# aikiriao/AAD

Hardware: AMD Instinct MI355X
Metric: Msamples/s encode+decode, 48 kHz stereo 4-bit (higher is better)
Workload: dtype int32

## Files before the change

### aad_amd/capi.py

```python
import ctypes as C
import os

import numpy as np


class AADApiResult:
    OK = 0
    INVALID_ARGUMENT = 1
    INVALID_FORMAT = 2
    INSUFFICIENT_BUFFER = 3
    INSUFFICIENT_DATA = 4
    PARAMETER_NOT_SET = 5
    NG = 6
    _names = {0: "OK", 1: "INVALID_ARGUMENT", 2: "INVALID_FORMAT", 3: "INSUFFICIENT_BUFFER",
              4: "INSUFFICIENT_DATA", 5: "PARAMETER_NOT_SET", 6: "NG"}

    @classmethod
    def name(cls, v):
        return cls._names.get(int(v), str(v))


class AADHeaderInfo(C.Structure):
    _fields_ = [("format_version", C.c_uint32), ("codec_version", C.c_uint32),
                ("num_channels", C.c_uint16), ("num_samples", C.c_uint32),
# ... 11 lines not shown
class AADHipStreamDesc(C.Structure):
    _fields_ = [("pcm_offset", C.c_uint64), ("data_offset", C.c_uint64),
                ("data_size", C.c_uint64), ("num_samples", C.c_uint32), ("reserved", C.c_uint32)]


class AADHipSegmentation(C.Structure):
    _fields_ = [("segment_blocks", C.c_uint32), ("warmup_blocks", C.c_uint32)]


class AADHipPlanarLayout(C.Structure):
    _fields_ = [("sample_type", C.c_int32), ("reserved", C.c_uint32), ("channel_stride", C.c_uint64)]


class AADHipPlanarOutput(C.Structure):
    _fields_ = [("sample_type", C.c_int32), ("reserved", C.c_uint32), ("stream_stride", C.c_uint64), ("channel_stride", C.c_uint64)]


class AADHipRowStats(C.Structure):
    _fields_ = [("sum_sq", C.c_uint64), ("sum_abs", C.c_uint64), ("max_abs", C.c_uint64), ("count", C.c_uint64)]


class AADHipLaneState(C.Structure):
    _fields_ = [("weight", C.c_int32 * 4), ("history", C.c_int32 * 4),
                ("stepsize_index", C.c_int32), ("quantize_error", C.c_int32)]


STREAM_DESC_DTYPE = np.dtype([("pcm_offset", "<u8"), ("data_offset", "<u8"), ("data_size", "<u8"),
                              ("num_samples", "<u4"), ("reserved", "<u4")])
ERROR_STATS_DTYPE = np.dtype([("rms_error", "<f8"), ("mean_abs_error", "<f8"), ("max_abs_error", "<f8")])
WINDOW_DTYPE = np.dtype([("stream", "<i8"), ("first_frame", "<i8")])
SAMPLE_INT16, SAMPLE_FLOAT32 = 0, 1
RECONSTRUCT_DECODED, RECONSTRUCT_RESIDUAL = 0, 1
OPTION_LANE_MAPPING, OPTION_TRIAL_LANES, OPTION_STAGING_THREADS, OPTION_TILE_KBYTES, OPTION_COMPARE_ORDER = 0, 1, 2, 3, 4
LANE_MAPPINGS = {"auto": 0, "dense": 1, "quad": 2, "quad-fused": 3, "dense-tiled": 4}
TRIAL_LANES = {"dual": 0, "single": 1}
LANE_STATE_DTYPE = np.dtype([("weight", "<i4", (4,)), ("history", "<i4", (4,)),
                             ("stepsize_index", "<i4"), ("quantize_error", "<i4")])

_PKG_DIR = os.path.dirname(os.path.abspath(__file__))
LIBRARY_PATH = os.environ.get("AAD_HIP_LIBRARY", os.path.join(_PKG_DIR, "libaad_hip.so"))

LEGACY_SYMBOLS = [
    "AADEncoder_CalculateBlockSize", "AADEncoder_EncodeHeader", "AADEncoder_CalculateWorkSize",
    "AADEncoder_Create", "AADEncoder_Destroy", "AADEncoder_SetEncodeParameter", "AADEncoder_EncodeWhole",
    "AADDecoder_DecodeHeader", "AADDecoder_CalculateWorkSize", "AADDecoder_Create", "AADDecoder_Destroy",
    "AADDecoder_SetHeader", "AADDecoder_DecodeBlock", "AADDecoder_DecodeWhole",
]
HIP_SYMBOLS = [
    "AADHip_GetDeviceCount", "AADHip_ContextCreate", "AADHip_ContextDestroy", "AADHip_ContextSynchronize",
    "AADHip_ContextLastError", "AADHip_ContextSignalNextRun", "AADHip_SignalNextRunSupported", "AADHip_ContextSetOption", "AADHip_CalculateEncodedSize", "AADHip_EncodePlanCreate",
    "AADHip_EncodePlanDestroy", "AADHip_EncodePlanRun", "AADHip_DecodePlanCreate", "AADHip_DecodePlanDestroy",
    "AADHip_DecodePlanRun", "AADHip_EncodeBatch", "AADHip_DecodeBatch",
    "AADHip_ReconstructPlanCreate", "AADHip_ReconstructPlanDestroy", "AADHip_ReconstructPlanRun",
    "AADHip_ReconstructBatch", "AADHip_SegmentedEncodePlanCreate", "AADHip_SegmentedEncodeBatch",
    "AADHip_SegmentedReconstructPlanCreate", "AADHip_SegmentedReconstructBatch",
    "AADHip_WindowDecodePlanCreate", "AADHip_WindowDecodePlanDestroy", "AADHip_WindowDecodePlanRun",
    "AADHip_PlanarEncodePlanCreate", "AADHip_PlanarEncodePlanRun",
    "AADHip_PlanarReconstructPlanCreate", "AADHip_PlanarReconstructPlanRun", "AADHip_PlanarReconstructPlanRunStats",
]
WAV_SYMBOLS = ["AADWav_ParseHeader", "AADWav_WriteHeader", "AADWav_ConvertToPcm16"]
SYNTH_SYMBOLS = ["AADSynth_Generate"]


class AADWavInfo(C.Structure):
    _fields_ = [("format_tag", C.c_uint16), ("num_channels", C.c_uint16), ("sampling_rate", C.c_uint32),
                ("bits_per_sample", C.c_uint16), ("num_samples", C.c_uint32), ("data_offset", C.c_uint64),
                ("data_size", C.c_uint64)]


def _declare_legacy(lib):
    u8p, i32pp = C.POINTER(C.c_uint8), C.POINTER(C.POINTER(C.c_int32))
    lib.AADEncoder_CalculateBlockSize.argtypes = [C.c_uint16, C.c_uint16, C.c_uint32,
                                                  C.POINTER(C.c_uint16), C.POINTER(C.c_uint32)]
    lib.AADEncoder_CalculateBlockSize.restype = C.c_int
    lib.AADEncoder_EncodeHeader.argtypes = [C.POINTER(AADHeaderInfo), u8p, C.c_uint32]
    lib.AADEncoder_EncodeHeader.restype = C.c_int
    lib.AADEncoder_CalculateWorkSize.argtypes = [C.c_uint16]
    lib.AADEncoder_CalculateWorkSize.restype = C.c_int32
    lib.AADEncoder_Create.argtypes = [C.c_uint16, C.c_void_p, C.c_int32]
    lib.AADEncoder_Create.restype = C.c_void_p
    lib.AADEncoder_Destroy.argtypes = [C.c_void_p]
    lib.AADEncoder_Destroy.restype = None
    lib.AADEncoder_SetEncodeParameter.argtypes = [C.c_void_p, C.POINTER(AADEncodeParameter)]
    lib.AADEncoder_SetEncodeParameter.restype = C.c_int
    lib.AADEncoder_EncodeWhole.argtypes = [C.c_void_p, i32pp, C.c_uint32, u8p, C.c_uint32, C.POINTER(C.c_uint32)]
    lib.AADEncoder_EncodeWhole.restype = C.c_int
    lib.AADDecoder_DecodeHeader.argtypes = [u8p, C.c_uint32, C.POINTER(AADHeaderInfo)]
    lib.AADDecoder_DecodeHeader.restype = C.c_int
    lib.AADDecoder_CalculateWorkSize.argtypes = []
    lib.AADDecoder_CalculateWorkSize.restype = C.c_int32
    lib.AADDecoder_Create.argtypes = [C.c_void_p, C.c_int32]
# ... 54 lines not shown
    lib.AADHip_DecodePlanCreate.argtypes = [vp, C.POINTER(AADHeaderInfo), C.c_int32, C.c_uint32, vp, C.POINTER(vp)]
    lib.AADHip_DecodePlanCreate.restype = C.c_int
    lib.AADHip_DecodePlanDestroy.argtypes = [vp]
    lib.AADHip_DecodePlanDestroy.restype = None
    lib.AADHip_DecodePlanRun.argtypes = [vp, vp, vp]
    lib.AADHip_DecodePlanRun.restype = C.c_int
    lib.AADHip_WindowDecodePlanCreate.argtypes = [vp, C.POINTER(AADHeaderInfo), C.c_int32, C.c_uint32, vp, C.POINTER(vp)]
    lib.AADHip_WindowDecodePlanCreate.restype = C.c_int
    lib.AADHip_WindowDecodePlanDestroy.argtypes = [vp]
    lib.AADHip_WindowDecodePlanDestroy.restype = None
    lib.AADHip_WindowDecodePlanRun.argtypes = [vp, vp, C.c_uint64, vp, C.c_uint32, C.c_int32, vp]
    lib.AADHip_WindowDecodePlanRun.restype = C.c_int
    lib.AADHip_EncodeBatch.argtypes = [vp, C.POINTER(AADEncodeParameter), C.c_uint32, vp, vp, vp, vp, vp, vp]
    lib.AADHip_EncodeBatch.restype = C.c_int
    lib.AADHip_DecodeBatch.argtypes = [vp, C.c_uint32, vp, vp, vp, vp, vp]
    lib.AADHip_DecodeBatch.restype = C.c_int
    lib.AADHip_ReconstructPlanCreate.argtypes = [vp, C.POINTER(AADEncodeParameter), C.c_uint32, vp, C.POINTER(vp)]
    lib.AADHip_ReconstructPlanCreate.restype = C.c_int
    lib.AADHip_ReconstructPlanDestroy.argtypes = [vp]
    lib.AADHip_ReconstructPlanDestroy.restype = None
    lib.AADHip_ReconstructPlanRun.argtypes = [vp, vp, vp, vp, C.c_int32, vp]
    lib.AADHip_ReconstructPlanRun.restype = C.c_int
    lib.AADHip_ReconstructBatch.argtypes = [vp, C.POINTER(AADEncodeParameter), C.c_uint32, vp, vp, C.c_int32, vp, vp]
    lib.AADHip_ReconstructBatch.restype = C.c_int
    lib.AADHip_SegmentedEncodeBatch.argtypes = [vp, C.POINTER(AADEncodeParameter), C.POINTER(AADHipSegmentation), C.c_uint32, vp, vp,
                                                vp, vp, vp]
    lib.AADHip_SegmentedEncodeBatch.restype = C.c_int
    lib.AADHip_SegmentedReconstructPlanCreate.argtypes = [vp, C.POINTER(AADEncodeParameter), C.POINTER(AADHipSegmentation), C.c_uint32,
                                                          vp, C.POINTER(vp)]
    lib.AADHip_SegmentedReconstructPlanCreate.restype = C.c_int
    lib.AADHip_SegmentedReconstructBatch.argtypes = [vp, C.POINTER(AADEncodeParameter), C.POINTER(AADHipSegmentation), C.c_uint32, vp,
                                                     vp, C.c_int32, vp, vp]
    lib.AADHip_SegmentedReconstructBatch.restype = C.c_int
    lib.AADWav_ParseHeader.argtypes = [vp, C.c_uint64, C.POINTER(AADWavInfo)]
    lib.AADWav_ParseHeader.restype = C.c_int
    lib.AADWav_WriteHeader.argtypes = [vp, C.c_uint32, C.c_uint16, C.c_uint32, C.c_uint32]
    lib.AADWav_WriteHeader.restype = C.c_int
    lib.AADWav_ConvertToPcm16.argtypes = [vp, C.c_uint16, C.c_uint64, vp]
    lib.AADWav_ConvertToPcm16.restype = C.c_int


def load_library(path=None, hip=True):
    path = path or LIBRARY_PATH
    if not os.path.exists(path):
        raise FileNotFoundError(
            "%s is missing - the HIP extension has not been built (run __graft_entry__.build())" % path)
    if hip:
        try:
            import torch
        except ImportError:
            pass
    lib = C.CDLL(path)
    _declare_legacy(lib)
    if hip:
        _declare_hip(lib)
    return lib


def make_parameter(channels, bits, max_block_size=1024, rate=48000, ms=False, trials=0):
    return AADEncodeParameter(num_channels=channels, sampling_rate=rate, bits_per_sample=bits,
                              max_block_size=max_block_size, ch_process_method=1 if ms else 0,
                              num_encode_trials=trials)


def _planar_pointers(planar):
    rows = (C.POINTER(C.c_int32) * planar.shape[0])()
# ... 88 lines not shown
```

### aad_amd/csrc/aad_hip_engine.hip

```cpp
#include <hip/hip_runtime.h>

#include <cstdio>
#include <cstdlib>
#include <cstring>
#include <algorithm>
#include <condition_variable>
#include <functional>
#include <mutex>
#include <new>
#include <thread>
#include <vector>

#include "../../include/aad_hip.h"
#include "aad_compare.hip.h"
#include "aad_launch.h"
#include "aad_decode.hip.h"
#include "aad_decode_window.hip.h"
#include "aad_encode.hip.h"
#include "aad_encode_launch.hip.h"
#include "aad_format.h"
#include "aad_hip_internal.h"
#include "aad_tiles.h"

namespace aad {
// ... 12 lines not shown
struct StagingPool {
  std::vector<std::thread> threads;
  std::mutex lock;
  std::condition_variable work, done;
  std::function<void(unsigned)> job;
  unsigned generation = 0, pending = 0;
  bool stop = false;
};

struct AADHipContext {
  int device;
  hipStream_t stream;
  bool owns_stream;
  char last_error[256];
  Staging in[2], out[2];
  hipEvent_t chunk_done[2];
  hipEvent_t piece_done[3];
  hipStream_t up_stream, down_stream;
  hipEvent_t uploaded[2], computed[2];
  bool have_events, have_pipeline;
  void *d_rc_in, *d_rc_out;
  size_t rc_in_capacity, rc_out_capacity;
  void *d_scratch;
  size_t scratch_capacity;
  int32_t *d_residual;
  uint64_t residual_capacity;
  uint8_t *d_trial;
  uint64_t trial_capacity;
  aad::LaunchSignal signal_next;
  bool signal_refused;
  aad::Device device_info;
  aad::Knobs knobs;
  int32_t compare_sequential;
  int64_t tile_bytes;
  void *d_state;
  size_t state_capacity;
  int32_t staging_threads;
  StagingPool *pool;
};

enum class EncodePlanKind {
  Frames,
  Rows,
  Reconstruct
};

struct AADHipEncodePlan {
  AADHipContext *ctx;
  EncodePlanKind kind;
  aad::EncodeRun run;
  void *d_table;
  uint64_t *d_out_base;
  uint32_t *d_stats_stream;
  uint64_t stats_records;
};

struct AADHipDecodePlan {
  AADHipContext *ctx;
  aad::DecodeArgs args;
  aad::StreamDesc *d_streams;
  uint64_t *d_prefix;
};

struct AADHipWindowDecodePlan {
  AADHipContext *ctx;
  aad::DecodeArgs args;
// ... 563 lines not shown
      if (ctx->d_trial) (void)hipFree(ctx->d_trial);
      if (ctx->d_state) (void)hipFree(ctx->d_state);
      if (ctx->owns_stream) (void)hipStreamDestroy(ctx->stream);
    }
  }
  delete ctx;
}

AADApiResult AADHip_ContextSynchronize(struct AADHipContext *ctx)
{
  if (ctx == nullptr) return AAD_APIRESULT_INVALID_ARGUMENT;
  DeviceGuard guard(ctx);
  if (!guard.ok) return AAD_APIRESULT_NG;
  return hip_ok(ctx, hipStreamSynchronize(ctx->stream), "hipStreamSynchronize") ? AAD_APIRESULT_OK : AAD_APIRESULT_NG;
}

const char *AADHip_ContextLastError(const struct AADHipContext *ctx) { return ctx ? ctx->last_error : ""; }

void AADHipInternal_ContextOptionsFromEnvironment(struct AADHipContext *ctx)
{
  static const char *const kMappings[] = {"auto", "dense", "quad", "quad-fused", "dense-tiled"};
  static const char *const kTrialLanes[] = {"dual", "single"};
  ctx->signal_refused = AADHip_SignalNextRunSupported() == 0;
  ctx->knobs.lane_mapping = option_from_env("AAD_HIP_MAPPING", kMappings, 5);
  ctx->knobs.trial_lanes = option_from_env("AAD_HIP_TRIAL_LANES", kTrialLanes, 2);
  const char *ring = getenv("AAD_HIP_ENCODE_RING"), *enc_pad = getenv("AAD_HIP_ENCODE_LDS_PAD");
  const char *dec_pad = getenv("AAD_HIP_DECODE_LDS_PAD"), *nt_min = getenv("AAD_HIP_DECODE_NT_MIN");
  ctx->knobs.encode_ring = ring != nullptr && ring[0] == '0' ? 0 : (ring != nullptr && ring[0] == '2' ? 2 : 1);
  ctx->knobs.encode_lds_pad = enc_pad ? atoi(enc_pad) : -1;
  ctx->knobs.decode_lds_pad = dec_pad ? atoi(dec_pad) : -1;
  ctx->knobs.decode_nt_min = nt_min ? (uint64_t)atoll(nt_min) : 0ull;
  static const char *const kCompareOrders[] = {"auto", "sequential"};
  ctx->compare_sequential = option_from_env("AAD_HIP_COMPARE_ORDER", kCompareOrders, 2);
  const char *threads = getenv("AAD_HIP_STAGING_THREADS");
  if (threads != nullptr && threads[0] >= '1' && threads[0] <= '8' && threads[1] == '\0') ctx->staging_threads = threads[0] - '0';
  const char *tile = getenv("AAD_HIP_TILE_KBYTES");
  if (tile != nullptr) {
    const long long v = atoll(tile);
    if (v > 0 && v <= 0x7FFFFFFF) ctx->tile_bytes = (int64_t)v << 10;
  }
}

int32_t AADHipInternal_ContextDevice(const struct AADHipContext *ctx) { return ctx->device; }

int32_t AADHip_SignalNextRunSupported(void)
{
  const char *v = getenv("ROC_SYSTEM_SCOPE_SIGNAL");
  return (v != nullptr && v[0] == '0' && v[1] == '\0') ? 0 : 1;
}

AADApiResult AADHip_ContextSignalNextRun(struct AADHipContext *ctx, void *hip_start_event, void *hip_stop_event)
{
  if (ctx == nullptr) return AAD_APIRESULT_INVALID_ARGUMENT;
  if (ctx->signal_refused && (hip_start_event != nullptr || hip_stop_event != nullptr)) {
    snprintf(ctx->last_error, sizeof(ctx->last_error),
             "AADHip_ContextSignalNextRun: refused, ROC_SYSTEM_SCOPE_SIGNAL=0 (device-scope completion signals: a wait on the "
             "run's event from another stream would never return); record an event behind the run instead");
    return AAD_APIRESULT_NG;
  }
  ctx->signal_next = aad::LaunchSignal{static_cast<hipEvent_t>(hip_start_event), static_cast<hipEvent_t>(hip_stop_event)};
  return AAD_APIRESULT_OK;
}

AADApiResult AADHip_ContextSetOption(struct AADHipContext *ctx, int32_t option, int32_t value)
{
  if (ctx == nullptr) return AAD_APIRESULT_INVALID_ARGUMENT;
  switch (option) {
    case AAD_HIP_OPTION_LANE_MAPPING:
      if (value < AAD_HIP_LANE_MAPPING_AUTO || value > AAD_HIP_LANE_MAPPING_DENSE_TILED) return AAD_APIRESULT_INVALID_ARGUMENT;
      ctx->knobs.lane_mapping = value;
      return AAD_APIRESULT_OK;
    case AAD_HIP_OPTION_TRIAL_LANES:
      if (value != AAD_HIP_TRIAL_LANES_DUAL && value != AAD_HIP_TRIAL_LANES_SINGLE) return AAD_APIRESULT_INVALID_ARGUMENT;
      ctx->knobs.trial_lanes = value;
      return AAD_APIRESULT_OK;
    case AAD_HIP_OPTION_COMPARE_ORDER:
      if (value != 0 && value != 1) return AAD_APIRESULT_INVALID_ARGUMENT;
      ctx->compare_sequential = value;
      return AAD_APIRESULT_OK;
    case AAD_HIP_OPTION_STAGING_THREADS:
      if (value < 0 || value > 8) return AAD_APIRESULT_INVALID_ARGUMENT;
      ctx->staging_threads = value;
      return AAD_APIRESULT_OK;
    case AAD_HIP_OPTION_TILE_KBYTES:
      if (value < 0) return AAD_APIRESULT_INVALID_ARGUMENT;
      ctx->tile_bytes = (int64_t)value << 10;
      return AAD_APIRESULT_OK;
    default:
      return AAD_APIRESULT_INVALID_ARGUMENT;
  }
}

uint64_t AADHip_CalculateEncodedSize(const struct AADEncodeParameter *parameter, uint32_t num_samples)
{
  AADHeaderInfo h;
  if (num_samples == 0) return 0;
  if (AADFormat_ParameterToHeader(parameter, num_samples, AAD_HIP_MAX_NUM_CHANNELS, &h) != AAD_APIRESULT_OK) return 0;
  if (!AADFormat_HeaderFieldsValid(&h, AAD_HIP_MAX_NUM_CHANNELS)) return 0;
  return AADFormat_EncodedSize(&h);
}


AADApiResult AADHip_EncodePlanCreate(struct AADHipContext *ctx, const struct AADEncodeParameter *parameter,
                                     uint32_t num_streams, const struct AADHipStreamDesc *streams,
                                     struct AADHipEncodePlan **plan)
{
  if (ctx == nullptr || parameter == nullptr || plan == nullptr || (num_streams != 0 && streams == nullptr))
    return AAD_APIRESULT_INVALID_ARGUMENT;
  *plan = nullptr;
  return encode_plan_create(ctx, parameter, nullptr, nullptr, nullptr, num_streams, streams, plan);
}

void AADHip_EncodePlanDestroy(struct AADHipEncodePlan *plan)
{
  if (plan == nullptr) return;
  DeviceGuard guard(plan->ctx);
  if (guard.ok) {
    (void)hipStreamSynchronize(plan->ctx->stream);
    (void)hipFree(plan->d_table);
// ... 1143 lines not shown
```

### aad_amd/csrc/aad_hip_internal.h

```cpp
#ifndef AAD_HIP_INTERNAL_H
#define AAD_HIP_INTERNAL_H

#include "../../include/aad_hip.h"

#ifdef __cplusplus
extern "C" {
#endif

AADApiResult AADHipInternal_DecodeHost(struct AADHipContext *context, const struct AADHeaderInfo *format,
                                       int32_t has_file_header, uint32_t num_streams,
                                       const uint8_t *const *data, const uint64_t *data_size,
                                       const uint32_t *num_samples, int16_t *const *pcm, uint32_t *decoded_frames);


void AADHipInternal_ContextOptionsFromEnvironment(struct AADHipContext *context);
int32_t AADHipInternal_ContextDevice(const struct AADHipContext *context);

AADApiResult AADHipInternal_EncodePlanar32(struct AADHipContext *context, const struct AADEncodeParameter *parameter,
                                           const int32_t *const *input, uint32_t num_samples, uint8_t *data,
                                           uint64_t data_capacity, uint64_t *output_size, struct AADHipLaneState *state);
AADApiResult AADHipInternal_DecodePlanar32(struct AADHipContext *context, const struct AADHeaderInfo *format,
                                           int32_t has_file_header, const uint8_t *data, uint64_t data_size,
                                           uint32_t want_frames, int32_t *const *buffer, uint32_t *decoded_frames);

#ifdef __cplusplus
}
#endif
#endif
```

### aad_amd/engine.py

```python
import ctypes as C

import numpy as np

from .capi import (AADApiResult, AADHeaderInfo, AADHipPlanarLayout, AADHipPlanarOutput, AADHipSegmentation, ApiError, ERROR_STATS_DTYPE, LANE_MAPPINGS, LANE_STATE_DTYPE,
                   OPTION_COMPARE_ORDER, OPTION_LANE_MAPPING, OPTION_STAGING_THREADS, OPTION_TILE_KBYTES, OPTION_TRIAL_LANES, RECONSTRUCT_DECODED, RECONSTRUCT_RESIDUAL,
                   SAMPLE_FLOAT32, SAMPLE_INT16, STREAM_DESC_DTYPE, TRIAL_LANES, WINDOW_DTYPE, load_library, make_parameter)


def _check(where, rc):
    if rc != AADApiResult.OK:
        raise ApiError(where, rc)


def _round_up(v, a):
    return (v + a - 1) // a * a


class Engine:

    def __init__(self, device=0, stream="torch", lib=None):
        import torch
        if not torch.cuda.is_available():
            raise RuntimeError("aad_amd.Engine needs a HIP device (torch.cuda.is_available() is False)")
        self.torch = torch
        self.lib = lib or load_library()
        self.device = int(device)
        torch.cuda.set_device(self.device)
        if stream == "torch":
            cur = torch.cuda.current_stream(self.device)
            self.stream = cur if cur.cuda_stream != 0 else torch.cuda.Stream(self.device)
        elif stream is None:
            self.stream = torch.cuda.Stream(self.device)
        else:
            self.stream = stream
        self._ctx = C.c_void_p()
        _check("AADHip_ContextCreate",
               self.lib.AADHip_ContextCreate(self.device, self.stream.cuda_stream, C.byref(self._ctx)))

# ... 555 lines not shown
        rc = self.runtime().hipEventCreateWithFlags(C.byref(self.handle), 0x0 if timing else 0x2)
        if rc != 0:
            raise RuntimeError("hipEventCreateWithFlags failed (%d)" % rc)

    def wait_on(self, stream):
        rc = self.runtime().hipStreamWaitEvent(C.c_void_p(stream.cuda_stream), self.handle, 0)
        if rc != 0:
            raise RuntimeError("hipStreamWaitEvent failed (%d)" % rc)

    def elapsed_ms(self, stop):
        ms = C.c_float()
        rc = self.runtime().hipEventElapsedTime(C.byref(ms), self.handle, stop.handle)
        if rc != 0:
            raise RuntimeError("hipEventElapsedTime failed (%d)" % rc)
        return float(ms.value)

    def synchronize(self):
        rc = self.runtime().hipEventSynchronize(self.handle)
        if rc != 0:
            raise RuntimeError("hipEventSynchronize failed (%d)" % rc)

    def close(self):
        if self.handle:
            self.runtime().hipEventDestroy(self.handle)
            self.handle = C.c_void_p()

    def __del__(self):
        try:
            self.close()
        except Exception:
            pass


class EncodeDecodePipeline:

    def __init__(self, enc_engine, dec_engine, param, streams, samples, ring=8):
        assert ring >= 2 and ring % 2 == 0
        assert enc_engine.stream.cuda_stream != dec_engine.stream.cuda_stream, "the two contexts need streams of their own"
        torch = enc_engine.torch
        self.torch, self.ring, self.k = torch, ring, 0
        self.enc_engine, self.dec_engine = enc_engine, dec_engine
        self.enc = enc_engine.uniform_encode_plan(param, streams, samples)
        self.images = [torch.zeros((streams, self.enc.stride), dtype=torch.uint8, device="cuda:%d" % enc_engine.device)
                       for _ in range(ring)]
        zero = torch.zeros((streams, samples, param.num_channels), dtype=torch.int16, device=self.images[0].device)
        self.enc.run(zero, self.images[0])
        torch.cuda.synchronize()
        self.header = parse_header(bytes(self.images[0][0, :31].cpu().numpy()))
        self.dec = dec_engine.uniform_decode_plan(self.header, streams, self.enc.stride, self.enc.image_size)
        self.encoded = [HipEvent() for _ in range(ring)]
        self.decoded = [torch.cuda.Event() for _ in range(ring)]

    def step(self, pcm, out, timing=None):
        k, ring = self.k, self.ring
        self.k += 1
        b = k % ring
        s_enc, s_dec = self.enc_engine.stream, self.dec_engine.stream
        if k >= ring and k % (ring // 2) == 0:
            s_enc.wait_event(self.decoded[(k - ring // 2 - 1) % ring])
        encoded = self.encoded[b] if timing is None else timing[1]
        self.enc_engine.signal_next(encoded, start=None if timing is None else timing[0])
        self.enc.run(pcm, self.images[b], None, ordered=False)
        encoded.wait_on(s_dec)
        if timing is not None:
            self.dec_engine.signal_next(timing[3], start=timing[2])
        self.dec.run(self.images[b], out, ordered=False)
        self.decoded[b].record(s_dec)
        return self.images[b]

    def close(self):
        self.torch.cuda.synchronize()
        self.enc.close()
        self.dec.close()
        for e in self.encoded:
            e.close()


def parse_header(data):
    if len(data) < 31 or data[:4] != b"AAD\x00":
        raise ApiError("parse_header", AADApiResult.INVALID_FORMAT)
    be = lambda o, n: int.from_bytes(data[o:o + n], "big")
    return AADHeaderInfo(format_version=be(4, 4), codec_version=be(8, 4), num_channels=be(12, 2),
                         num_samples=be(14, 4), sampling_rate=be(18, 4), bits_per_sample=be(22, 2),
                         block_size=be(24, 2), num_samples_per_block=be(26, 4), ch_process_method=data[30])


__all__ = ["Engine", "EncodePlan", "PlanarEncodePlan", "PlanarReconstructPlan", "DecodePlan", "WindowDecodePlan", "EncodeDecodePipeline", "parse_header", "make_parameter", "LANE_STATE_DTYPE", "rmse", "snr_db", "select_least_bits"]
```

### include/aad_hip.h

```cpp
#ifndef AAD_HIP_H_INCLUDED
#define AAD_HIP_H_INCLUDED

#include <stdint.h>
#include "aad.h"
#include "aad_encoder.h"

#define AAD_HIP_MAX_NUM_CHANNELS 8

struct AADHipContext;
struct AADHipEncodePlan;
struct AADHipDecodePlan;

struct AADHipStreamDesc {
  uint64_t pcm_offset;
  uint64_t data_offset;
  uint64_t data_size;
  uint32_t num_samples;
  uint32_t reserved;
};

struct AADHipLaneState {
  int32_t weight[4];
  int32_t history[4];
  int32_t stepsize_index;
  int32_t quantize_error;
};

#ifdef __cplusplus
extern "C" {
#endif

int32_t AADHip_GetDeviceCount(void);

AADApiResult AADHip_ContextCreate(int32_t device_index, void *hip_stream, struct AADHipContext **context);
void AADHip_ContextDestroy(struct AADHipContext *context);
AADApiResult AADHip_ContextSynchronize(struct AADHipContext *context);
const char *AADHip_ContextLastError(const struct AADHipContext *context);

AADApiResult AADHip_ContextSignalNextRun(struct AADHipContext *context, void *hip_start_event, void *hip_stop_event);
int32_t AADHip_SignalNextRunSupported(void);

enum AADHipOption {
  AAD_HIP_OPTION_LANE_MAPPING = 0,
  AAD_HIP_OPTION_TRIAL_LANES = 1,
  AAD_HIP_OPTION_STAGING_THREADS = 2,
  AAD_HIP_OPTION_TILE_KBYTES = 3,
  AAD_HIP_OPTION_COMPARE_ORDER = 4
};
enum AADHipLaneMapping {
  AAD_HIP_LANE_MAPPING_AUTO = 0,
  AAD_HIP_LANE_MAPPING_DENSE = 1,
  AAD_HIP_LANE_MAPPING_QUAD = 2,
  AAD_HIP_LANE_MAPPING_QUAD_FUSED = 3,
  AAD_HIP_LANE_MAPPING_DENSE_TILED = 4
};
enum AADHipTrialLanes {
  AAD_HIP_TRIAL_LANES_DUAL = 0,
  AAD_HIP_TRIAL_LANES_SINGLE = 1
};
AADApiResult AADHip_ContextSetOption(struct AADHipContext *context, int32_t option, int32_t value);

uint64_t AADHip_CalculateEncodedSize(const struct AADEncodeParameter *parameter, uint32_t num_samples);


AADApiResult AADHip_EncodePlanCreate(
    struct AADHipContext *context, const struct AADEncodeParameter *parameter,
    uint32_t num_streams, const struct AADHipStreamDesc *streams,
    struct AADHipEncodePlan **plan);
void AADHip_EncodePlanDestroy(struct AADHipEncodePlan *plan);

AADApiResult AADHip_EncodePlanRun(
    struct AADHipEncodePlan *plan, const int16_t *device_pcm, uint8_t *device_data,
    struct AADHipLaneState *device_state);


struct AADHipSegmentation {
  uint32_t segment_blocks;
  uint32_t warmup_blocks;
};
AADApiResult AADHip_SegmentedEncodePlanCreate(
// ... 49 lines not shown
    struct AADHipLaneState *device_state);


struct AADHipPlanarOutput {
  int32_t sample_type;
  uint32_t reserved;
  uint64_t stream_stride;
  uint64_t channel_stride;
};
AADApiResult AADHip_PlanarReconstructPlanCreate(
    struct AADHipContext *context, const struct AADEncodeParameter *parameter,
    const struct AADHipPlanarLayout *input, const struct AADHipPlanarOutput *output,
    const struct AADHipSegmentation *segmentation,
    uint32_t num_streams, const struct AADHipStreamDesc *streams,
    struct AADHipEncodePlan **plan);
AADApiResult AADHip_PlanarReconstructPlanRun(
    struct AADHipEncodePlan *plan, const void *device_samples, uint8_t *device_data, void *device_out,
    struct AADHipLaneState *device_state);


struct AADHipRowStats {
  uint64_t sum_sq;
  uint64_t sum_abs;
  uint64_t max_abs;
  uint64_t count;
};
AADApiResult AADHip_PlanarReconstructPlanRunStats(
    struct AADHipEncodePlan *plan, const void *device_samples, uint8_t *device_data,
    void *device_out,
    struct AADHipLaneState *device_state,
    struct AADHipRowStats *device_stats);


AADApiResult AADHip_EncodeBatch(
    struct AADHipContext *context, const struct AADEncodeParameter *parameter,
    uint32_t num_streams, const int16_t *const *pcm, const uint32_t *num_samples,
    uint8_t *const *data, const uint64_t *data_capacity, uint64_t *output_size,
    struct AADHipLaneState *state);

AADApiResult AADHip_SegmentedEncodeBatch(
    struct AADHipContext *context, const struct AADEncodeParameter *parameter,
    const struct AADHipSegmentation *segmentation,
    uint32_t num_streams, const int16_t *const *pcm, const uint32_t *num_samples,
    uint8_t *const *data, const uint64_t *data_capacity, uint64_t *output_size);

AADApiResult AADHip_DecodeBatch(
    struct AADHipContext *context, uint32_t num_streams,
    const uint8_t *const *data, const uint64_t *data_size,
    int16_t *const *pcm, const uint32_t *pcm_capacity_frames, uint32_t *decoded_frames);


enum AADHipReconstructOutput {
  AAD_HIP_RECONSTRUCT_DECODED = 0,
  AAD_HIP_RECONSTRUCT_RESIDUAL = 1
};

struct AADHipErrorStats {
  double rms_error;
  double mean_abs_error;
  double max_abs_error;
};

struct AADHipReconstructPlan;

AADApiResult AADHip_ReconstructPlanCreate(
    struct AADHipContext *context, const struct AADEncodeParameter *parameter,
// ... 30 lines not shown
```

Before: 103,300.

## Move encode/decode pipeline into C and add alternating schedule option

Replaces the Python-driven encode/decode pipeline step with a native AADHip_Pipeline object that issues the waits, signals and plan runs from C, removing per-step Python and torch event overhead. It also adds an alternating schedule where both contexts take turns doing encode and decode with a chain of decode-to-decode waits, beside the existing split schedule. The default schedule stays split unless the environment or option selects alternating. Risks include the event ordering being wrong in edge cases and extra ABI surface.

```diff
diff --git a/aad_amd/capi.py b/aad_amd/capi.py
--- a/aad_amd/capi.py
+++ b/aad_amd/capi.py
@@ -67,6 +67,8 @@
 SAMPLE_INT16, SAMPLE_FLOAT32 = 0, 1
 RECONSTRUCT_DECODED, RECONSTRUCT_RESIDUAL = 0, 1
 OPTION_LANE_MAPPING, OPTION_TRIAL_LANES, OPTION_STAGING_THREADS, OPTION_TILE_KBYTES, OPTION_COMPARE_ORDER = 0, 1, 2, 3, 4
+OPTION_PIPELINE_SCHEDULE = 5
+PIPELINE_SCHEDULES = {"alternating": 0, "split": 1}
 LANE_MAPPINGS = {"auto": 0, "dense": 1, "quad": 2, "quad-fused": 3, "dense-tiled": 4}
 TRIAL_LANES = {"dual": 0, "single": 1}
 LANE_STATE_DTYPE = np.dtype([("weight", "<i4", (4,)), ("history", "<i4", (4,)),
@@ -92,6 +94,8 @@
     "AADHip_WindowDecodePlanCreate", "AADHip_WindowDecodePlanDestroy", "AADHip_WindowDecodePlanRun",
     "AADHip_PlanarEncodePlanCreate", "AADHip_PlanarEncodePlanRun",
     "AADHip_PlanarReconstructPlanCreate", "AADHip_PlanarReconstructPlanRun", "AADHip_PlanarReconstructPlanRunStats",
+    "AADHip_PipelineCreate", "AADHip_PipelineStep", "AADHip_PipelineHeader", "AADHip_PipelineImage", "AADHip_PipelineSchedule",
+    "AADHip_PipelineDestroy",
 ]
 WAV_SYMBOLS = ["AADWav_ParseHeader", "AADWav_WriteHeader", "AADWav_ConvertToPcm16"]
 SYNTH_SYMBOLS = ["AADSynth_Generate"]
@@ -212,6 +216,18 @@
     lib.AADHip_SegmentedReconstructBatch.argtypes = [vp, C.POINTER(AADEncodeParameter), C.POINTER(AADHipSegmentation), C.c_uint32, vp,
                                                      vp, C.c_int32, vp, vp]
     lib.AADHip_SegmentedReconstructBatch.restype = C.c_int
+    lib.AADHip_PipelineCreate.argtypes = [vp, vp, C.POINTER(AADEncodeParameter), C.c_uint32, C.c_uint32, C.c_uint32, C.POINTER(vp)]
+    lib.AADHip_PipelineCreate.restype = C.c_int
+    lib.AADHip_PipelineStep.argtypes = [vp, vp, vp, vp, C.POINTER(vp)]
+    lib.AADHip_PipelineStep.restype = C.c_int
+    lib.AADHip_PipelineHeader.argtypes = [vp, C.POINTER(AADHeaderInfo), C.POINTER(C.c_uint64), C.POINTER(C.c_uint64)]
+    lib.AADHip_PipelineHeader.restype = C.c_int
+    lib.AADHip_PipelineImage.argtypes = [vp, C.c_uint32, C.POINTER(vp)]
+    lib.AADHip_PipelineImage.restype = C.c_int
+    lib.AADHip_PipelineSchedule.argtypes = [vp]
+    lib.AADHip_PipelineSchedule.restype = C.c_int32
+    lib.AADHip_PipelineDestroy.argtypes = [vp]
+    lib.AADHip_PipelineDestroy.restype = None
     lib.AADWav_ParseHeader.argtypes = [vp, C.c_uint64, C.POINTER(AADWavInfo)]
     lib.AADWav_ParseHeader.restype = C.c_int
     lib.AADWav_WriteHeader.argtypes = [vp, C.c_uint32, C.c_uint16, C.c_uint32, C.c_uint32]
diff --git a/aad_amd/csrc/aad_hip_engine.hip b/aad_amd/csrc/aad_hip_engine.hip
--- a/aad_amd/csrc/aad_hip_engine.hip
+++ b/aad_amd/csrc/aad_hip_engine.hip
@@ -68,6 +68,7 @@
   aad::Device device_info;
   aad::Knobs knobs;
   int32_t compare_sequential;
+  int32_t pipeline_schedule;
   int64_t tile_bytes;
   void *d_state;
   size_t state_capacity;
@@ -697,6 +698,9 @@
   ctx->knobs.decode_nt_min = nt_min ? (uint64_t)atoll(nt_min) : 0ull;
   static const char *const kCompareOrders[] = {"auto", "sequential"};
   ctx->compare_sequential = option_from_env("AAD_HIP_COMPARE_ORDER", kCompareOrders, 2);
+  static const char *const kPipelineSchedules[] = {"split", "alternating"};
+  ctx->pipeline_schedule = option_from_env("AAD_HIP_PIPELINE_SCHEDULE", kPipelineSchedules, 2) == 1 ? AAD_HIP_PIPELINE_SCHEDULE_ALTERNATING
+                                                                                                    : AAD_HIP_PIPELINE_SCHEDULE_SPLIT;
   const char *threads = getenv("AAD_HIP_STAGING_THREADS");
   if (threads != nullptr && threads[0] >= '1' && threads[0] <= '8' && threads[1] == '\0') ctx->staging_threads = threads[0] - '0';
   const char *tile = getenv("AAD_HIP_TILE_KBYTES");
@@ -707,6 +711,12 @@
 }
 
 int32_t AADHipInternal_ContextDevice(const struct AADHipContext *ctx) { return ctx->device; }
+void *AADHipInternal_ContextStream(const struct AADHipContext *ctx) { return ctx->stream; }
+int32_t AADHipInternal_ContextPipelineSchedule(const struct AADHipContext *ctx) { return ctx->pipeline_schedule; }
+void AADHipInternal_ContextSetLastError(struct AADHipContext *ctx, const char *text)
+{
+  snprintf(ctx->last_error, sizeof(ctx->last_error), "%s", text);
+}
 
 int32_t AADHip_SignalNextRunSupported(void)
 {
@@ -750,6 +760,10 @@
     case AAD_HIP_OPTION_TILE_KBYTES:
       if (value < 0) return AAD_APIRESULT_INVALID_ARGUMENT;
       ctx->tile_bytes = (int64_t)value << 10;
+      return AAD_APIRESULT_OK;
+    case AAD_HIP_OPTION_PIPELINE_SCHEDULE:
+      if (value != AAD_HIP_PIPELINE_SCHEDULE_ALTERNATING && value != AAD_HIP_PIPELINE_SCHEDULE_SPLIT) return AAD_APIRESULT_INVALID_ARGUMENT;
+      ctx->pipeline_schedule = value;
       return AAD_APIRESULT_OK;
     default:
       return AAD_APIRESULT_INVALID_ARGUMENT;
diff --git a/aad_amd/csrc/aad_hip_internal.h b/aad_amd/csrc/aad_hip_internal.h
--- a/aad_amd/csrc/aad_hip_internal.h
+++ b/aad_amd/csrc/aad_hip_internal.h
@@ -16,6 +16,10 @@
 void AADHipInternal_ContextOptionsFromEnvironment(struct AADHipContext *context);
 int32_t AADHipInternal_ContextDevice(const struct AADHipContext *context);
 
+void *AADHipInternal_ContextStream(const struct AADHipContext *context);
+int32_t AADHipInternal_ContextPipelineSchedule(const struct AADHipContext *context);
+void AADHipInternal_ContextSetLastError(struct AADHipContext *context, const char *text);
+
 AADApiResult AADHipInternal_EncodePlanar32(struct AADHipContext *context, const struct AADEncodeParameter *parameter,
                                            const int32_t *const *input, uint32_t num_samples, uint8_t *data,
                                            uint64_t data_capacity, uint64_t *output_size, struct AADHipLaneState *state);
diff --git a/aad_amd/csrc/aad_pipeline.hip b/aad_amd/csrc/aad_pipeline.hip
--- /dev/null
+++ b/aad_amd/csrc/aad_pipeline.hip
@@ -0,0 +1,214 @@
+#include <hip/hip_runtime.h>
+
+#include <cstdio>
+#include <new>
+#include <vector>
+
+#include "../../include/aad_hip.h"
+#include "aad_format.h"
+#include "aad_hip_internal.h"
+#include "aad_pipeline_schedule.h"
+
+static_assert((int32_t)aad::kScheduleAlternating == AAD_HIP_PIPELINE_SCHEDULE_ALTERNATING &&
+                  (int32_t)aad::kScheduleSplit == AAD_HIP_PIPELINE_SCHEDULE_SPLIT,
+              "enum AADHipPipelineSchedule");
+
+struct AADHipPipeline {
+  AADHipContext *ctx[2];
+  hipStream_t stream[2];
+  int device;
+  int32_t schedule;
+  uint32_t ring;
+  uint64_t k;
+  AADHipEncodePlan *enc[2];
+  AADHipDecodePlan *dec[2];
+  uint8_t *images;
+  uint64_t slot_bytes, image_size, image_stride;
+  std::vector<hipEvent_t> encoded, decoded;
+  hipEvent_t last_decode_stop;
+  AADHeaderInfo header;
+};
+
+namespace {
+
+struct OnDevice {
+  int prev = -1;
+  bool ok;
+  explicit OnDevice(int device)
+  {
+    if (hipGetDevice(&prev) != hipSuccess) prev = -1;
+    ok = prev == device || hipSetDevice(device) == hipSuccess;
+    if (prev == device) prev = -1;
+  }
+  ~OnDevice()
+  {
+    if (prev >= 0) (void)hipSetDevice(prev);
+  }
+};
+
+AADApiResult fail(AADHipPipeline *p, const char *what, hipError_t e)
+{
+  char text[200];
+  snprintf(text, sizeof(text), "pipeline: %s: %s", what, hipGetErrorString(e));
+  AADHipInternal_ContextSetLastError(p->ctx[0], text);
+  return AAD_APIRESULT_NG;
+}
+
+void uniform_table(std::vector<AADHipStreamDesc> *t, uint32_t n, uint64_t pcm_stride, uint64_t data_stride, uint64_t data_size,
+                   uint32_t num_samples)
+{
+  t->resize(n);
+  for (uint32_t i = 0; i < n; i++) (*t)[i] = AADHipStreamDesc{i * pcm_stride, i * data_stride, data_size, num_samples, 0};
+}
+
+}
+
+extern "C" {
+
+void AADHip_PipelineDestroy(struct AADHipPipeline *p)
+{
+  if (p == nullptr) return;
+  OnDevice here(p->device);
+  if (here.ok) {
+    (void)hipStreamSynchronize(p->stream[0]);
+    (void)hipStreamSynchronize(p->stream[1]);
+  }
+  for (int c = 0; c < 2; c++) {
+    AADHip_EncodePlanDestroy(p->enc[c]);
+    AADHip_DecodePlanDestroy(p->dec[c]);
+  }
+  if (here.ok) {
+    for (hipEvent_t e : p->encoded) (void)hipEventDestroy(e);
+    for (hipEvent_t e : p->decoded) (void)hipEventDestroy(e);
+    if (p->images) (void)hipFree(p->images);
+  }
+  delete p;
+}
+
+AADApiResult AADHip_PipelineCreate(struct AADHipContext *a, struct AADHipContext *b, const struct AADEncodeParameter *parameter,
+                                   uint32_t num_streams, uint32_t num_samples, uint32_t ring, struct AADHipPipeline **pipeline)
+{
+  if (pipeline == nullptr) return AAD_APIRESULT_INVALID_ARGUMENT;
+  *pipeline = nullptr;
+  if (a == nullptr || b == nullptr || a == b || parameter == nullptr || num_streams == 0 || num_samples == 0 || !aad::pipeline_ring_ok(ring))
+    return AAD_APIRESULT_INVALID_ARGUMENT;
+  if (AADHipInternal_ContextStream(a) == AADHipInternal_ContextStream(b) || AADHipInternal_ContextDevice(a) != AADHipInternal_ContextDevice(b))
+    return AAD_APIRESULT_INVALID_ARGUMENT;
+  AADHeaderInfo h;
+  AADApiResult rc = AADFormat_ParameterToHeader(parameter, num_samples, AAD_HIP_MAX_NUM_CHANNELS, &h);
+  if (rc != AAD_APIRESULT_OK) return rc;
+  const uint64_t size = AADHip_CalculateEncodedSize(parameter, num_samples);
+  if (size == 0) return AAD_APIRESULT_INVALID_FORMAT;
+  if (AADHip_SignalNextRunSupported() == 0) {
+    AADHipInternal_ContextSetLastError(a, "pipeline: refused, ROC_SYSTEM_SCOPE_SIGNAL=0 (a wait on a kernel's completion signal from "
+                                          "another stream would never return)");
+    return AAD_APIRESULT_NG;
+  }
+
+  AADHipPipeline *p = new (std::nothrow) AADHipPipeline();
+  if (p == nullptr) return AAD_APIRESULT_NG;
+  p->ctx[0] = a;
+  p->ctx[1] = b;
+  for (int c = 0; c < 2; c++) {
+    p->stream[c] = static_cast<hipStream_t>(AADHipInternal_ContextStream(p->ctx[c]));
+    p->enc[c] = nullptr;
+    p->dec[c] = nullptr;
+  }
+  p->device = AADHipInternal_ContextDevice(a);
+  p->schedule = AADHipInternal_ContextPipelineSchedule(a);
+  p->ring = ring;
+  p->k = 0;
+  p->images = nullptr;
+  p->last_decode_stop = nullptr;
+  p->header = h;
+  p->image_size = size;
+  p->image_stride = (size + 63) / 64 * 64;
+  p->slot_bytes = p->image_stride * num_streams;
+
+  std::vector<AADHipStreamDesc> enc_table, dec_table;
+  uniform_table(&enc_table, num_streams, (uint64_t)num_samples * h.num_channels, p->image_stride, p->image_stride, num_samples);
+  uniform_table(&dec_table, num_streams, (uint64_t)num_samples * h.num_channels, p->image_stride, p->image_size, num_samples);
+  const bool split = p->schedule == aad::kScheduleSplit;
+  for (int c = 0; c < 2 && rc == AAD_APIRESULT_OK; c++) {
+    if (!split || c == 0) rc = AADHip_EncodePlanCreate(p->ctx[c], parameter, num_streams, enc_table.data(), &p->enc[c]);
+    if (rc == AAD_APIRESULT_OK && (!split || c == 1))
+      rc = AADHip_DecodePlanCreate(p->ctx[c], &h, 1, num_streams, dec_table.data(), &p->dec[c]);
+  }
+  OnDevice here(p->device);
+  if (rc == AAD_APIRESULT_OK && !here.ok) rc = AAD_APIRESULT_NG;
+  if (rc == AAD_APIRESULT_OK) {
+    hipError_t e = hipMalloc((void **)&p->images, p->slot_bytes * ring);
+    if (e == hipSuccess) e = hipMemsetAsync(p->images, 0, p->slot_bytes * ring, p->stream[0]);
+    if (e == hipSuccess) e = hipStreamSynchronize(p->stream[0]);
+    for (uint32_t i = 0; i < 2 * ring && e == hipSuccess; i++) {
+      hipEvent_t ev = nullptr;
+      e = hipEventCreateWithFlags(&ev, hipEventDisableTiming);
+      if (e == hipSuccess) (i < ring ? p->encoded : p->decoded).push_back(ev);
+    }
+    if (e != hipSuccess) rc = fail(p, "hipMalloc / hipEventCreate", e);
+  }
+  if (rc != AAD_APIRESULT_OK) {
+    AADHip_PipelineDestroy(p);
+    return rc;
+  }
+  *pipeline = p;
+  return AAD_APIRESULT_OK;
+}
+
+AADApiResult AADHip_PipelineStep(struct AADHipPipeline *p, const int16_t *device_pcm, int16_t *device_out, void *const *events,
+                                 uint8_t **device_image)
+{
+  if (p == nullptr || device_pcm == nullptr || device_out == nullptr) return AAD_APIRESULT_INVALID_ARGUMENT;
+  const aad::PipelineStep s = aad::pipeline_step(p->k, p->ring, p->schedule);
+  const uint32_t ce = s.encode_context, cd = s.decode_context;
+  uint8_t *image = p->images + (uint64_t)s.slot * p->slot_bytes;
+  hipEvent_t timing[4] = {nullptr, nullptr, nullptr, nullptr};
+  for (int i = 0; events != nullptr && i < 4; i++) timing[i] = static_cast<hipEvent_t>(events[i]);
+  OnDevice here(p->device);
+  if (!here.ok) return AAD_APIRESULT_NG;
+  hipError_t e;
+  AADApiResult rc;
+
+  if (s.encode_waits_decode != aad::kNoStep &&
+      (e = hipStreamWaitEvent(p->stream[ce], p->decoded[(uint64_t)s.encode_waits_decode % p->ring], 0)) != hipSuccess)
+    return fail(p, "hipStreamWaitEvent", e);
+  const hipEvent_t encode_stop = timing[1] != nullptr ? timing[1] : (s.arms_encode ? p->encoded[s.slot] : nullptr);
+  if ((rc = AADHip_ContextSignalNextRun(p->ctx[ce], timing[0], encode_stop)) != AAD_APIRESULT_OK) return rc;
+  if ((rc = AADHip_EncodePlanRun(p->enc[ce], device_pcm, image, nullptr)) != AAD_APIRESULT_OK) return rc;
+
+  if (s.decode_waits_encode != aad::kNoStep && (e = hipStreamWaitEvent(p->stream[cd], encode_stop, 0)) != hipSuccess)
+    return fail(p, "hipStreamWaitEvent", e);
+  if (s.decode_waits_decode != aad::kNoStep && (e = hipStreamWaitEvent(p->stream[cd], p->last_decode_stop, 0)) != hipSuccess)
+    return fail(p, "hipStreamWaitEvent", e);
+  const hipEvent_t decode_stop = timing[3] != nullptr ? timing[3] : (s.arms_decode ? p->decoded[s.slot] : nullptr);
+  if ((rc = AADHip_ContextSignalNextRun(p->ctx[cd], timing[2], decode_stop)) != AAD_APIRESULT_OK) return rc;
+  if ((rc = AADHip_DecodePlanRun(p->dec[cd], image, device_out)) != AAD_APIRESULT_OK) return rc;
+  if (p->schedule == aad::kScheduleSplit && s.decode_awaited && decode_stop != p->decoded[s.slot] &&
+      (e = hipEventRecord(p->decoded[s.slot], p->stream[cd])) != hipSuccess)
+    return fail(p, "hipEventRecord", e);
+  p->last_decode_stop = decode_stop;
+  p->k++;
+  if (device_image != nullptr) *device_image = image;
+  return AAD_APIRESULT_OK;
+}
+
+AADApiResult AADHip_PipelineHeader(const struct AADHipPipeline *p, struct AADHeaderInfo *header, uint64_t *image_size,
+                                   uint64_t *image_stride)
+{
+  if (p == nullptr) return AAD_APIRESULT_INVALID_ARGUMENT;
+  if (header != nullptr) *header = p->header;
+  if (image_size != nullptr) *image_size = p->image_size;
+  if (image_stride != nullptr) *image_stride = p->image_stride;
+  return AAD_APIRESULT_OK;
+}
+
+AADApiResult AADHip_PipelineImage(const struct AADHipPipeline *p, uint32_t slot, uint8_t **device_image)
+{
+  if (p == nullptr || device_image == nullptr || slot >= p->ring) return AAD_APIRESULT_INVALID_ARGUMENT;
+  *device_image = p->images + (uint64_t)slot * p->slot_bytes;
+  return AAD_APIRESULT_OK;
+}
+
+int32_t AADHip_PipelineSchedule(const struct AADHipPipeline *p) { return p != nullptr ? p->schedule : -1; }
+
+}
diff --git a/aad_amd/csrc/aad_pipeline_schedule.h b/aad_amd/csrc/aad_pipeline_schedule.h
--- /dev/null
+++ b/aad_amd/csrc/aad_pipeline_schedule.h
@@ -0,0 +1,48 @@
+#ifndef AAD_PIPELINE_SCHEDULE_H
+#define AAD_PIPELINE_SCHEDULE_H
+
+#include <stdint.h>
+
+namespace aad {
+
+enum PipelineSchedule : int32_t { kScheduleAlternating = 0, kScheduleSplit = 1 };
+
+constexpr int64_t kNoStep = -1;
+
+struct PipelineStep {
+  uint32_t encode_context, decode_context;
+  uint32_t slot;
+  int64_t encode_waits_decode;
+  int64_t decode_waits_encode;
+  int64_t decode_waits_decode;
+  bool arms_encode, arms_decode, decode_awaited;
+};
+
+inline bool pipeline_ring_ok(uint32_t ring) { return ring >= 2 && ring % 2 == 0; }
+
+inline PipelineStep pipeline_step(uint64_t k, uint32_t ring, int32_t schedule)
+{
+  PipelineStep s;
+  s.slot = (uint32_t)(k % ring);
+  s.encode_waits_decode = s.decode_waits_encode = s.decode_waits_decode = kNoStep;
+  if (schedule == kScheduleSplit) {
+    const uint64_t half = ring / 2;
+    s.encode_context = 0;
+    s.decode_context = 1;
+    if (k >= ring && k % half == 0) s.encode_waits_decode = (int64_t)(k - half - 1);
+    s.decode_waits_encode = (int64_t)k;
+    s.arms_encode = true;
+    s.arms_decode = true;
+    s.decode_awaited = (k + 1) % half == 0;
+  } else {
+    s.encode_context = s.decode_context = (uint32_t)(k & 1);
+    if (k >= 1) s.decode_waits_decode = (int64_t)(k - 1);
+    s.arms_encode = false;
+    s.arms_decode = s.decode_awaited = true;
+  }
+  return s;
+}
+
+}
+
+#endif
diff --git a/aad_amd/engine.py b/aad_amd/engine.py
--- a/aad_amd/engine.py
+++ b/aad_amd/engine.py
@@ -3,7 +3,7 @@
 import numpy as np
 
 from .capi import (AADApiResult, AADHeaderInfo, AADHipPlanarLayout, AADHipPlanarOutput, AADHipSegmentation, ApiError, ERROR_STATS_DTYPE, LANE_MAPPINGS, LANE_STATE_DTYPE,
-                   OPTION_COMPARE_ORDER, OPTION_LANE_MAPPING, OPTION_STAGING_THREADS, OPTION_TILE_KBYTES, OPTION_TRIAL_LANES, RECONSTRUCT_DECODED, RECONSTRUCT_RESIDUAL,
+                   OPTION_COMPARE_ORDER, OPTION_LANE_MAPPING, OPTION_PIPELINE_SCHEDULE, OPTION_STAGING_THREADS, OPTION_TILE_KBYTES, OPTION_TRIAL_LANES, PIPELINE_SCHEDULES, RECONSTRUCT_DECODED, RECONSTRUCT_RESIDUAL,
                    SAMPLE_FLOAT32, SAMPLE_INT16, STREAM_DESC_DTYPE, TRIAL_LANES, WINDOW_DTYPE, load_library, make_parameter)
 
 
@@ -625,48 +625,62 @@
             pass
 
 
+class _DeviceRows:
+
+    def __init__(self, pointer, rows, cols):
+        self.__cuda_array_interface__ = {"shape": (int(rows), int(cols)), "typestr": "|u1", "data": (int(pointer), False),
+                                         "strides": None, "version": 2}
+
+
+class _PipelineImages:
+
+    def __init__(self, image_size, stride):
+        self.image_size, self.stride = image_size, stride
+
+
 class EncodeDecodePipeline:
 
-    def __init__(self, enc_engine, dec_engine, param, streams, samples, ring=8):
+    def __init__(self, enc_engine, dec_engine, param, streams, samples, ring=8, schedule=None):
         assert ring >= 2 and ring % 2 == 0
         assert enc_engine.stream.cuda_stream != dec_engine.stream.cuda_stream, "the two contexts need streams of their own"
         torch = enc_engine.torch
-        self.torch, self.ring, self.k = torch, ring, 0
+        self.torch, self.ring, self.lib = torch, ring, enc_engine.lib
         self.enc_engine, self.dec_engine = enc_engine, dec_engine
-        self.enc = enc_engine.uniform_encode_plan(param, streams, samples)
-        self.images = [torch.zeros((streams, self.enc.stride), dtype=torch.uint8, device="cuda:%d" % enc_engine.device)
-                       for _ in range(ring)]
-        zero = torch.zeros((streams, samples, param.num_channels), dtype=torch.int16, device=self.images[0].device)
-        self.enc.run(zero, self.images[0])
-        torch.cuda.synchronize()
-        self.header = parse_header(bytes(self.images[0][0, :31].cpu().numpy()))
-        self.dec = dec_engine.uniform_decode_plan(self.header, streams, self.enc.stride, self.enc.image_size)
-        self.encoded = [HipEvent() for _ in range(ring)]
-        self.decoded = [torch.cuda.Event() for _ in range(ring)]
+        if schedule is not None:
+            _check("AADHip_ContextSetOption",
+                   self.lib.AADHip_ContextSetOption(enc_engine._ctx, OPTION_PIPELINE_SCHEDULE, PIPELINE_SCHEDULES[schedule]))
+        self.handle = C.c_void_p()
+        _check("AADHip_PipelineCreate",
+               self.lib.AADHip_PipelineCreate(enc_engine._ctx, dec_engine._ctx, C.byref(param), streams, samples, ring, C.byref(self.handle)))
+        self.header = AADHeaderInfo()
+        size, stride = C.c_uint64(), C.c_uint64()
+        _check("AADHip_PipelineHeader", self.lib.AADHip_PipelineHeader(self.handle, C.byref(self.header), C.byref(size), C.byref(stride)))
+        self.enc = _PipelineImages(int(size.value), int(stride.value))
+        self.schedule = {v: k for k, v in PIPELINE_SCHEDULES.items()}[self.lib.AADHip_PipelineSchedule(self.handle)]
+        self.images, self._slot = [], {}
+        for b in range(ring):
+            ptr = C.c_void_p()
+            _check("AADHip_PipelineImage", self.lib.AADHip_PipelineImage(self.handle, b, C.byref(ptr)))
+            self.images.append(torch.as_tensor(_DeviceRows(ptr.value, streams, stride.value), device="cuda:%d" % enc_engine.device))
+            self._slot[ptr.value] = b
 
     def step(self, pcm, out, timing=None):
-        k, ring = self.k, self.ring
-        self.k += 1
-        b = k % ring
-        s_enc, s_dec = self.enc_engine.stream, self.dec_engine.stream
-        if k >= ring and k % (ring // 2) == 0:
-            s_enc.wait_event(self.decoded[(k - ring // 2 - 1) % ring])
-        encoded = self.encoded[b] if timing is None else timing[1]
-        self.enc_engine.signal_next(encoded, start=None if timing is None else timing[0])
-        self.enc.run(pcm, self.images[b], None, ordered=False)
-        encoded.wait_on(s_dec)
-        if timing is not None:
-            self.dec_engine.signal_next(timing[3], start=timing[2])
-        self.dec.run(self.images[b], out, ordered=False)
-        self.decoded[b].record(s_dec)
-        return self.images[b]
+        events = None if timing is None else (C.c_void_p * 4)(*[e.handle for e in timing])
+        image = C.c_void_p()
+        _check("AADHip_PipelineStep", self.lib.AADHip_PipelineStep(self.handle, pcm.data_ptr(), out.data_ptr(), events, C.byref(image)))
+        return self.images[self._slot[image.value]]
 
     def close(self):
-        self.torch.cuda.synchronize()
-        self.enc.close()
-        self.dec.close()
-        for e in self.encoded:
-            e.close()
+        if self.handle:
+            self.lib.AADHip_PipelineDestroy(self.handle)
+            self.handle = C.c_void_p()
+            self.images = []
+
+    def __del__(self):
+        try:
+            self.close()
+        except Exception:
+            pass
 
 
 def parse_header(data):
diff --git a/include/aad_hip.h b/include/aad_hip.h
--- a/include/aad_hip.h
+++ b/include/aad_hip.h
@@ -45,7 +45,12 @@
   AAD_HIP_OPTION_TRIAL_LANES = 1,
   AAD_HIP_OPTION_STAGING_THREADS = 2,
   AAD_HIP_OPTION_TILE_KBYTES = 3,
-  AAD_HIP_OPTION_COMPARE_ORDER = 4
+  AAD_HIP_OPTION_COMPARE_ORDER = 4,
+  AAD_HIP_OPTION_PIPELINE_SCHEDULE = 5
+};
+enum AADHipPipelineSchedule {
+  AAD_HIP_PIPELINE_SCHEDULE_ALTERNATING = 0,
+  AAD_HIP_PIPELINE_SCHEDULE_SPLIT = 1
 };
 enum AADHipLaneMapping {
   AAD_HIP_LANE_MAPPING_AUTO = 0,
@@ -161,6 +166,20 @@
     struct AADHipRowStats *device_stats);
 
 
+struct AADHipPipeline;
+AADApiResult AADHip_PipelineCreate(
+    struct AADHipContext *context_a, struct AADHipContext *context_b, const struct AADEncodeParameter *parameter,
+    uint32_t num_streams, uint32_t num_samples, uint32_t ring, struct AADHipPipeline **pipeline);
+AADApiResult AADHip_PipelineStep(
+    struct AADHipPipeline *pipeline, const int16_t *device_pcm, int16_t *device_out, void *const *events,
+    uint8_t **device_image);
+AADApiResult AADHip_PipelineHeader(
+    const struct AADHipPipeline *pipeline, struct AADHeaderInfo *header, uint64_t *image_size, uint64_t *image_stride);
+AADApiResult AADHip_PipelineImage(const struct AADHipPipeline *pipeline, uint32_t slot, uint8_t **device_image);
+int32_t AADHip_PipelineSchedule(const struct AADHipPipeline *pipeline);
+void AADHip_PipelineDestroy(struct AADHipPipeline *pipeline);
+
+
 AADApiResult AADHip_EncodeBatch(
     struct AADHipContext *context, const struct AADEncodeParameter *parameter,
     uint32_t num_streams, const int16_t *const *pcm, const uint32_t *num_samples,
```

After: 101,700. 0.984x the previous value.
